# pyannote/pyannote-audio

Measured on AMD Instinct MI355X. Metric: audio-hours/sec (real-time factor) for speaker-diarization-3.1 pipeline, higher is better.
Workload: dtype f32

## Files before the change

include/pyannote_amd.h:

```cpp
#ifndef PYANNOTE_AMD_H
#define PYANNOTE_AMD_H

#include <stddef.h>
#include <stdint.h>

#ifdef __cplusplus
extern "C" {
#endif

int pa_version(void);
const char* pa_last_error(void);

void pa_prof_enable(int on);
size_t pa_prof_report(char* buf, size_t cap);

#define PA_MAX_LSTM_LAYERS 8
#define PA_MAX_LINEAR 4

typedef struct pa_seg_weights {
  int32_t sinc_stride;
  int32_t lstm_layers;
  int32_t lstm_hidden;
  int32_t lstm_bidir;
  int32_t num_linear;
// ... 71 lines not shown
  int32_t bottleneck;
  const float* fb_window;
  const float* fb_tw256;
  const float* fb_tw512;
  const float* fb_mel_w;
  const int32_t* fb_mel_lo;
  const int32_t* fb_mel_hi;
  const float* stem_w;
  const float* stem_shift;
  const float* blk_w1[PA_MAX_RES_BLOCKS];
  const float* blk_shift1[PA_MAX_RES_BLOCKS];
  const float* blk_w2[PA_MAX_RES_BLOCKS];
  const float* blk_shift2[PA_MAX_RES_BLOCKS];
  const float* blk_u1[PA_MAX_RES_BLOCKS];
  const float* blk_u2[PA_MAX_RES_BLOCKS];
  const float* blk_wsc[PA_MAX_RES_BLOCKS];
  const float* blk_shiftsc[PA_MAX_RES_BLOCKS];
  const float* blk_w3[PA_MAX_RES_BLOCKS];
  const float* blk_shift3[PA_MAX_RES_BLOCKS];
  const float* seg1_w;
  const float* seg1_b;
  const float* blk_v1[PA_MAX_RES_BLOCKS];
  const float* blk_v2[PA_MAX_RES_BLOCKS];
  int32_t fb_center_kernel;
} pa_emb_weights;

int pa_emb_num_fbank_frames(int num_samples);
int pa_emb_num_pool_frames(const pa_emb_weights* w, int num_samples);
size_t pa_emb_workspace_bytes(const pa_emb_weights* w, int num_chunks, int num_samples, int num_masks);
int pa_emb_forward(const pa_emb_weights* w, const float* wav, int64_t wav_len, int64_t chunk_stride,
                   int num_chunks, int num_samples, const float* masks, int num_masks, int mask_frames,
                   const int32_t* nearest_idx, float* emb, void* workspace, size_t workspace_bytes,
                   void* stream);

size_t pa_emb_ragged_workspace_bytes(const pa_emb_weights* w, int num_utterances, int max_samples);
int pa_emb_forward_ragged(const pa_emb_weights* w, const float* wav, int64_t wav_len, const int64_t* offsets,
                          const int32_t* lengths, int num_utterances, int max_samples, const float* masks, float* emb,
                          void* workspace, size_t workspace_bytes, void* stream);

size_t pa_emb_calibrate_workspace_bytes(const pa_emb_weights* w, int num_chunks, int num_samples);
int pa_emb_calibrate_winograd(const pa_emb_weights* w, const float* wav, int64_t wav_len, int64_t chunk_stride,
                              int num_chunks, int num_samples, float* report, float* emb, void* workspace,
                              size_t workspace_bytes, void* stream);
int pa_absmax_diff(const float* got, const float* ref, long n, float* out2, void* stream);

int pa_fbank(const float* wav, long wav_len, long chunk_stride, int B, int N, const float* window,
             const float* tw256, const float* tw512, const float* mel_w, const int* mel_lo,
             const int* mel_hi, int nmel, float* out, int center, void* stream);
int pa_fbank_center_span(const float* fb, int B, int T, int nmel, int kernel, float* out, void* stream);
int pa_resnet_stem(const float* fbank, int B, int T, int F, const float* w9, const float* shift,
                   float* out, void* stream);
int pa_conv3x3(const float* X, int B, int H, int W, int cin, const float* Wg, const float* shift,
               const float* R, float* Y, int cout, int stride, int relu, void* stream);
int pa_winograd_pack_host(const float* conv_weight ,
                          const float* bn_scale , int cout, int cin,
                          float* U_slabs );
int pa_conv3x3_wino(const float* X, int B, int H, int W, int cin, const float* U, const float* shift,
                    const float* R, float* Y, int cout, int relu, void* stream);
int pa_winograd4_pack_host(const float* conv_weight ,
                           const float* bn_scale , int cout, int cin,
                           float* U_slabs );
int pa_conv3x3_wino4(const float* X, int B, int H, int W, int cin, const float* U, const float* shift,
                     const float* R, float* Y, int cout, int relu, void* stream);
int pa_conv3x3_wino4_rows(const float* X, int B, int H, int W, int cin, const float* U, const float* shift,
                          const float* R, float* Y, int cout, int relu, int rows, void* stream);
int pa_conv3x3_wino_rows(const float* X, int B, int H, int W, int cin, const float* U, const float* shift,
                         const float* R, float* Y, int cout, int relu, int y_first, void* stream);
int pa_stats_pool(const float* feat, int B, int Fh, int Tp, int C, const float* masks, int S, int Fm,
                  const int* nearest_idx, float* stats, void* stream);
int pa_fbank_ragged(const float* wav, long wav_len, const int64_t* offsets, const int32_t* lengths, int B,
                    int max_samples, const float* window, const float* tw256, const float* tw512, const float* mel_w,
                    const int* mel_lo, const int* mel_hi, int nmel, float* out, void* stream);
int pa_zero_tail_cols(float* x, int B, int H, int W, int C, const int32_t* lengths, int halvings, void* stream);
int pa_stats_pool_ragged(const float* feat, int B, int Fh, int W, int C, const int32_t* lengths, int halvings,
                         const float* masks, int ld_masks, float* stats, void* stream);

#define PA_W2V_MAX_CONV 8
#define PA_W2V_MAX_LAYERS 24
typedef struct pa_w2v_layer {
  const float* qk_w;
  const float* qk_b;
  const float* v_w;
  const float* out_w;
  const float* out_b;
  const float* ln1_g;
  const float* ln1_b;
  const float* ff1_w;
  const float* ff1_b;
  const float* ff2_w;
  const float* ff2_b;
  const float* ln2_g;
  const float* ln2_b;
  const float* gate_w;
  const float* gate_b;
  const float* gate_const;
} pa_w2v_layer;

typedef struct pa_sser_weights {
  int32_t num_conv;
  int32_t conv_channels[PA_W2V_MAX_CONV];
  int32_t conv_kernel[PA_W2V_MAX_CONV];
  int32_t conv_stride[PA_W2V_MAX_CONV];
  int32_t extractor_layer_norm;
  int32_t embed_dim, num_layers, num_heads, ff_dim, layer_norm_first;
  int32_t pos_kernel, pos_groups;
  int32_t wavlm;
// ... 238 lines not shown
```

pyannote-audio_amd/csrc/emb_forward.cpp:

```cpp
#include "forward_common.h"

namespace {

struct EmbPlan {
  int B, N, T, F, S;
  int Hs[5], Ws[5];
  size_t fbank, act[4], stats, total, act_elems;
  size_t t2_off, gather_off;
};

inline bool prefer_wino4(int H, int W, int cin) {
  auto up = [](int a, int b) { return (long)((a + b - 1) / b) * b; };
  long p4 = up(H, 4) * up(W, 64);
  const long p4_lin = up(H, 4) * up(W, 4);
  if (p4_lin * 120 <= p4 * 100) p4 = p4_lin * 120 / 100;
  long p2 = up(H, 8) * up(W, 32);
  if (up(H, 4) * up(W, 64) < p2) p2 = up(H, 4) * up(W, 64);
  if (up(H, 2) * up(W, 128) < p2) p2 = up(H, 2) * up(W, 128);
  const long gain = cin >= 256 ? 130 : 122;
  return p4 * 100 <= p2 * gain;
}

bool make_plan(const pa_emb_weights* w, int B, int N, int S, EmbPlan* p, bool calib = false) {
  if (N < 400) return false;
  p->B = B;
  p->N = N;
  p->S = S < 1 ? 1 : S;
  p->T = 1 + (N - 400) / 160;
  p->F = w->num_mel;
  p->Hs[0] = p->F;
  p->Ws[0] = p->T;
  for (int l = 0; l < w->num_layers; ++l) {
    const int s = l == 0 ? 1 : 2;
    p->Hs[l + 1] = (p->Hs[l] - 1) / s + 1;
    p->Ws[l + 1] = (p->Ws[l] - 1) / s + 1;
  }
  pa::Bump ws;
  p->fbank = ws.take((size_t)B * p->T * p->F);
  const int ex = w->bottleneck ? 4 : 1;
  p->act_elems = (size_t)B * p->Hs[0] * p->Ws[0] * w->planes[0] * ex;
  for (int i = 0; i < 3; ++i) p->act[i] = ws.take(p->act_elems);
  p->t2_off = p->gather_off = 0;
  if (w->bottleneck) {
    size_t t1 = 0, t2 = 0, g = 0;
    int cin = w->planes[0];
    for (int l = 0; l < w->num_layers; ++l) {
      const size_t planes = w->planes[l];
      const size_t in_px = (size_t)B * p->Hs[l == 0 ? 1 : l] * p->Ws[l == 0 ? 1 : l];
      const size_t out_px = (size_t)B * p->Hs[l + 1] * p->Ws[l + 1];
      t1 = t1 > in_px * planes ? t1 : in_px * planes;
      t2 = t2 > out_px * planes ? t2 : out_px * planes;
      if (l > 0) g = g > out_px * cin ? g : out_px * cin;
      cin = 4 * (int)planes;
// ... 50 lines not shown
    pa::set_error("pa_emb_forward: workspace too small (%zu < %zu bytes)", workspace_bytes,
                  p.total * sizeof(float));
    return 3;
  }
  float* ws = (float*)workspace;
  const int B = p.B;

  const int span = w->fb_center_kernel;
  if (ragged && span != 0) {
    pa::set_error("pa_emb_forward_ragged: fbank_centering_span checkpoints run one launch sequence per length");
    return 3;
  }
  if (ragged)
    PA_RUN(pa_fbank_ragged(wav, wav_len, offsets, lengths, B, p.N, w->fb_window, w->fb_tw256, w->fb_tw512, w->fb_mel_w,
                           w->fb_mel_lo, w->fb_mel_hi, w->num_mel, ws + p.fbank, stream));
  else
    PA_RUN(pa_fbank(wav, wav_len, chunk_stride, B, p.N, w->fb_window, w->fb_tw256, w->fb_tw512, w->fb_mel_w,
                    w->fb_mel_lo, w->fb_mel_hi, w->num_mel, ws + p.fbank, span == 0 ? 1 : 0, stream));
  auto zero_tail = [&](float* X, int l, int C) -> int {
    return ragged ? pa_zero_tail_cols(X, B, p.Hs[l], p.Ws[l], C, lengths, l > 0 ? l - 1 : 0, stream) : 0;
  };
  float* cur = ws + p.act[0];
  float* f1 = ws + p.act[1];
  float* f2 = ws + p.act[2];
  const float* feats = ws + p.fbank;
  if (span != 0) {
    PA_RUN(pa_fbank_center_span(ws + p.fbank, B, p.T, p.F, span, f1, stream));
    feats = f1;
  }
  PA_RUN(pa_resnet_stem(feats, B, p.T, p.F, w->stem_w, w->stem_shift, cur, stream));
  if (!w->bottleneck) PA_RUN(zero_tail(cur, 0, w->planes[0]));

  auto conv_s1 = [&](const float* X, int H, int W, int ci, const float* v, const float* u, const float* wd,
                     const float* shift, const float* R, float* Y, int co, int slot) -> int {
    if (calib != nullptr) {
      float* scratch = ws + p.act[3];
      float* rep = calib + 4 * slot;
      const long n = (long)B * H * W * co;
      int r = pa_conv3x3(X, B, H, W, ci, wd, shift, R, Y, co, 1, 1, stream);
      if (r == 0 && v != nullptr) {
        r = pa_conv3x3_wino4(X, B, H, W, ci, v, shift, R, scratch, co, 1, stream);
        if (r == 0) r = pa_absmax_diff(scratch, Y, n, rep, stream);
      }
      if (r == 0 && u != nullptr) {
        r = pa_conv3x3_wino(X, B, H, W, ci, u, shift, R, scratch, co, 1, stream);
        if (r == 0) r = pa_absmax_diff(scratch, Y, n, rep + 2, stream);
      }
      return r;
    }
    if (v != nullptr && prefer_wino4(H, W, ci)) return pa_conv3x3_wino4(X, B, H, W, ci, v, shift, R, Y, co, 1, stream);
    if (u != nullptr) return pa_conv3x3_wino(X, B, H, W, ci, u, shift, R, Y, co, 1, stream);
    return pa_conv3x3(X, B, H, W, ci, wd, shift, R, Y, co, 1, 1, stream);
  };

  int blk = 0;
  int cin = w->planes[0];
  if (w->bottleneck) {
    float* nxt = f1;
    float* sc = f2;
    float* tmp = ws + p.act[3];
    for (int l = 0; l < w->num_layers; ++l) {
      const int planes = w->planes[l], cout = 4 * planes;
      for (int i = 0; i < w->num_blocks[l]; ++i, ++blk) {
        if (blk >= PA_MAX_RES_BLOCKS) {
          pa::set_error("pa_emb_forward: more than %d residual blocks", PA_MAX_RES_BLOCKS);
          return 3;
        }
        const int stride = (i == 0 && l > 0) ? 2 : 1;
        const int H = stride == 2 ? p.Hs[l] : p.Hs[l + 1], W = stride == 2 ? p.Ws[l] : p.Ws[l + 1];
        const int Ho = p.Hs[l + 1], Wo = p.Ws[l + 1];
        float* t1 = tmp;
        float* t2 = tmp + p.t2_off;
        PA_RUN(pa_gemm_tn_ex(cur, cin, w->blk_w1[blk], cin, w->blk_shift1[blk], nullptr, t1, planes, B * H * W,
                             planes, cin, 2, 0, stream));
        PA_RUN(zero_tail(t1, stride == 2 ? l : l + 1, planes));
        if (stride == 1 && w->blk_u2[blk] != nullptr)
          PA_RUN(pa_conv3x3_wino(t1, B, H, W, planes, w->blk_u2[blk], w->blk_shift2[blk], nullptr, t2, planes, 1,
                                 stream));
        else
          PA_RUN(pa_conv3x3(t1, B, H, W, planes, w->blk_w2[blk], w->blk_shift2[blk], nullptr, t2, planes, stride,
                            1, stream));
        const float* res = cur;
        if (w->blk_wsc[blk] != nullptr) {
          if (stride == 2)
            PA_RUN(pa_gemm_tn_s2(cur, B, H, W, cin, w->blk_wsc[blk], cin, w->blk_shiftsc[blk], sc, cout, cout, stream));
          else
            PA_RUN(pa_gemm_tn_ex(cur, cin, w->blk_wsc[blk], cin, w->blk_shiftsc[blk], nullptr, sc, cout,
                                 B * Ho * Wo, cout, cin, 0, 0, stream));
          res = sc;
        } else if (stride != 1 || cin != cout) {
          pa::set_error("pa_emb_forward: block %d needs a shortcut conv but none was given", blk);
          return 3;
        }
        PA_RUN(pa_gemm_tn_ex(t2, planes, w->blk_w3[blk], planes, w->blk_shift3[blk], res, nxt, cout, B * Ho * Wo,
                             cout, planes, 2, 0, stream));
        float* t = cur;
        cur = nxt;
        nxt = t;
        cin = cout;
      }
    }
  } else
  for (int l = 0; l < w->num_layers; ++l) {
    const int cout = w->planes[l];
    for (int i = 0; i < w->num_blocks[l]; ++i, ++blk) {
      if (blk >= PA_MAX_RES_BLOCKS) {
        pa::set_error("pa_emb_forward: more than %d residual blocks", PA_MAX_RES_BLOCKS);
        return 3;
      }
      const int stride = (i == 0 && l > 0) ? 2 : 1;
      const int H = stride == 2 ? p.Hs[l] : p.Hs[l + 1], W = stride == 2 ? p.Ws[l] : p.Ws[l + 1];
      const int Ho = p.Hs[l + 1], Wo = p.Ws[l + 1];
      if (w->blk_wsc[blk] != nullptr) {
        PA_RUN(pa_conv3x3(cur, B, H, W, cin, w->blk_w1[blk], w->blk_shift1[blk], nullptr, f1, cout, stride,
                          1, stream));
        PA_RUN(zero_tail(f1, l + 1, cout));
        const size_t q = (size_t)B * Ho * Wo * cin;
        float* R = f2 + pa::Bump::align(q);
        if (stride == 2)
          PA_RUN(pa_gemm_tn_s2(cur, B, H, W, cin, w->blk_wsc[blk], cin, w->blk_shiftsc[blk], R, cout, cout, stream));
        else
          PA_RUN(pa_gemm_tn(cur, cin, w->blk_wsc[blk], cin, w->blk_shiftsc[blk], R, cout, B * Ho * Wo, cout, cin, 0, 0,
                            stream));
        PA_RUN(conv_s1(f1, Ho, Wo, cout, w->blk_v2[blk], w->blk_u2[blk], w->blk_w2[blk], w->blk_shift2[blk], R, cur,
                       cout, 2 * blk + 1));
        PA_RUN(zero_tail(cur, l + 1, cout));
      } else {
        if (stride != 1 || cin != cout) {
          pa::set_error("pa_emb_forward: block %d needs a shortcut conv but none was given", blk);
          return 3;
        }
        PA_RUN(conv_s1(cur, H, W, cin, w->blk_v1[blk], w->blk_u1[blk], w->blk_w1[blk], w->blk_shift1[blk], nullptr, f1,
                       cout, 2 * blk));
        PA_RUN(zero_tail(f1, l + 1, cout));
        PA_RUN(conv_s1(f1, H, W, cout, w->blk_v2[blk], w->blk_u2[blk], w->blk_w2[blk], w->blk_shift2[blk], cur, f2,
                       cout, 2 * blk + 1));
        PA_RUN(zero_tail(f2, l + 1, cout));
        float* t = cur;
        cur = f2;
        f2 = t;
      }
      cin = cout;
    }
  }
  const int L = w->num_layers;
  const int S = p.S;
  const int cfin = w->planes[L - 1] * (w->bottleneck ? 4 : 1);
  if (ragged)
    PA_RUN(pa_stats_pool_ragged(cur, B, p.Hs[L], p.Ws[L], cfin, lengths, L - 1, masks, p.Ws[L], ws + p.stats, stream));
  else
    PA_RUN(pa_stats_pool(cur, B, p.Hs[L], p.Ws[L], cfin, masks, S, mask_frames, nearest_idx, ws + p.stats, stream));
  const int D2 = 2 * cfin * p.Hs[L];
  PA_RUN(pa_gemm_tn(ws + p.stats, D2, w->seg1_w, D2, w->seg1_b, emb, w->embed_dim, B * S, w->embed_dim, D2,
                    0, 0, stream));
  return 0;
}

extern "C" {

int pa_emb_forward(const pa_emb_weights* w, const float* wav, int64_t wav_len, int64_t chunk_stride,
                   int num_chunks, int num_samples, const float* masks, int num_masks, int mask_frames,
                   const int32_t* nearest_idx, float* emb, void* workspace, size_t workspace_bytes,
                   void* stream) {
  return emb_forward_impl(w, wav, wav_len, chunk_stride, num_chunks, num_samples, masks, num_masks, mask_frames,
                          nearest_idx, emb, workspace, workspace_bytes, stream, nullptr);
}

size_t pa_emb_ragged_workspace_bytes(const pa_emb_weights* w, int num_utterances, int max_samples) {
  EmbPlan p;
  if (!make_plan(w, num_utterances, max_samples, 1, &p)) return 0;
  return p.total * sizeof(float);
}

int pa_emb_forward_ragged(const pa_emb_weights* w, const float* wav, int64_t wav_len, const int64_t* offsets,
// ... 30 lines not shown
```

pyannote-audio_amd/csrc/emb_resnet.hip:

```cpp
#include "common.h"

namespace pa {

constexpr int STEM_TS = 64;
constexpr int STEM_LD = STEM_TS + 3;

__global__ __launch_bounds__(256) void k_stem(const float* __restrict__ fb, int T, int F,
                                              const float* __restrict__ w9,
                                              const float* __restrict__ shift,
                                              float* __restrict__ out) {
  extern __shared__ float xs[];
  const int b = blockIdx.y, t0 = blockIdx.x * STEM_TS;
  const int tid = threadIdx.x;
  for (int i = tid; i < 2 * STEM_LD; i += 256) xs[(i < STEM_LD ? 0 : (F + 1) * STEM_LD - STEM_LD) + i] = 0.f;
  const int n = (STEM_TS + 2) * F;
  for (int i0 = 0; i0 < n; i0 += 8 * 256) {
    float v[8];
#pragma unroll
    for (int k = 0; k < 8; ++k) {
      const int i = i0 + tid + 256 * k;
      const int tt = i / F, ff = i - tt * F, t = t0 + tt - 1;
      v[k] = (i < n && t >= 0 && t < T) ? fb[((long)b * T + t) * F + ff] : 0.f;
    }
#pragma unroll
// ... 24 lines not shown
  float* o = out + ((long)b * F * T + t0 + pl) * 32 + q4;
  for (int f = 0; f < F; ++f) {
#pragma unroll
    for (int h = 0; h < 2; ++h)
#pragma unroll
      for (int dt = 0; dt < 3; ++dt) x2[h][dt] = xs[(f + 2) * STEM_LD + pl + 32 * h + dt];
    float* of = o + (long)f * T * 32;
#pragma unroll
    for (int h = 0; h < 2; ++h) {
      float acc[4];
#pragma unroll
      for (int c = 0; c < 4; ++c) acc[c] = 0.f;
#pragma unroll
      for (int dt = 0; dt < 3; ++dt)
#pragma unroll
        for (int c = 0; c < 4; ++c) acc[c] = fmaf(x0[h][dt], w[dt][c], acc[c]);
#pragma unroll
      for (int dt = 0; dt < 3; ++dt)
#pragma unroll
        for (int c = 0; c < 4; ++c) acc[c] = fmaf(x1[h][dt], w[3 + dt][c], acc[c]);
#pragma unroll
      for (int dt = 0; dt < 3; ++dt)
#pragma unroll
        for (int c = 0; c < 4; ++c) acc[c] = fmaf(x2[h][dt], w[6 + dt][c], acc[c]);
      float4 o4;
      o4.x = fmaxf(acc[0] + sh[0], 0.f);
      o4.y = fmaxf(acc[1] + sh[1], 0.f);
      o4.z = fmaxf(acc[2] + sh[2], 0.f);
      o4.w = fmaxf(acc[3] + sh[3], 0.f);
      if (h == 0 ? ok0 : ok1) *reinterpret_cast<float4*>(of + 32 * 32 * h) = o4;
    }
#pragma unroll
    for (int h = 0; h < 2; ++h)
#pragma unroll
      for (int dt = 0; dt < 3; ++dt) {
        x0[h][dt] = x1[h][dt];
        x1[h][dt] = x2[h][dt];
      }
  }
}

constexpr int CB = 16;
constexpr int CLD = CB + 4;

template <int S, int TH, int TWT>
struct ConvGeom {
  static constexpr int TW = 32 * TWT;
  static constexpr int PH = (TH - 1) * S + 3;
  static constexpr int PW = (TW - 1) * S + 3;
  static constexpr int PWH = ((TW + 1 + 3) / 8) * 8 + 4;
  static constexpr int PATCH = S == 1 ? PH * PW * CLD : PH * 2 * PWH * CLD;
};

template <int S, int TH, int TWT, int BN, bool HAS_R>
__global__ __launch_bounds__(256, 2) void k_conv3x3(const float* __restrict__ X, int H, int W, int CIN,
                                                    const float* __restrict__ Wg,
                                                    const float* __restrict__ shift,
                                                    const float* __restrict__ R, float* __restrict__ Y,
                                                    int Ho, int Wo, int COUT, int relu, int tiles_w,
                                                    int tiles_hw, int n_tiles, int total_tiles, int xranges,
                                                    int* __restrict__ counters) {
  using G = ConvGeom<S, TH, TWT>;
  constexpr int MT = TH * TWT;
  constexpr int MPW = MT / 4;
  constexpr int NT = BN / 32;
  static_assert(MT % 4 == 0, "M-tiles must split over 4 waves");
  extern __shared__ __attribute__((aligned(16))) float smem[];
  float* patch = smem;
  float* wts = smem + G::PATCH;

  const int tid = threadIdx.x, lane = tid & 63, wv = tid >> 6;
  const int li = lane & 31, kh = lane >> 5;
  constexpr int NPF4 = G::PH * G::PW * (CB / 4);
  constexpr int NP = (NPF4 + 255) / 256;
  constexpr int NWF4 = 9 * BN * (CB / 4);
  constexpr int NW = (NWF4 + 255) / 256;
  constexpr int OOB = (int)0x80000000;

  struct Tile {
    int b, n0, y0, x0;
  };
  const int num_pb = total_tiles / n_tiles;
  auto pair_of = [&](int t) {
    return xranges ? (t & 7) * ((num_pb + 7) >> 3) + (t >> 3) / n_tiles : ((t >> 3) / n_tiles) * 8 + (t & 7);
  };
  auto decode = [&](int t) {
    Tile q;
    const int pb = pair_of(t);
    q.n0 = (((t >> 3) % n_tiles)) * BN;
    const int pix = pb % tiles_hw;
    q.b = pb / tiles_hw;
    q.y0 = (pix / tiles_w) * TH;
    q.x0 = (pix % tiles_w) * G::TW;
    return q;
  };
  auto resolve = [&](const TileQueue& tqq, int r) {
    for (;;) {
      const int t = tq_resolve(tqq, r);
      if (t < 0 || pair_of(t) < num_pb) return t;
      r = tq_claim_own(tqq);
    }
  };
  u32x4 rp[NP], rw[NW];
  constexpr bool HOIST = S == 2;
  struct Offs {
    int p[NP];
  };
  int offw[NW];
#pragma unroll
  for (int e = 0; e < NW; ++e) {
    const int i = tid + 256 * e;
    const int c4 = i & 3, rn = i >> 2;
    const int tap = rn / BN, n = rn % BN;
    offw[e] = (NWF4 % 256 == 0 || i < NWF4) ? ((tap * COUT + n) * CIN + 4 * c4) * 4 : OOB;
  }
  auto tile_offsets = [&](const Tile& q, Offs& o) {
#pragma unroll
    for (int e = 0; e < NP; ++e) {
      const int i = tid + 256 * e;
      const int c4 = i & 3, pp = i >> 2;
      const int py = pp / G::PW, px = pp % G::PW;
      const int iy = q.y0 * S - 1 + py, ix = q.x0 * S - 1 + px;
      o.p[e] = ((NPF4 % 256 == 0 || i < NPF4) && iy >= 0 && iy < H && ix >= 0 && ix < W)
                   ? ((iy * W + ix) * CIN + 4 * c4) * 4
                   : OOB;
    }
  };
  auto gload = [&](const Tile& q, const Offs& o, int c0) {
    const __amdgpu_buffer_rsrc_t xsrd = __builtin_amdgcn_make_buffer_rsrc(
        const_cast<float*>(X + (long)q.b * H * W * CIN), 0, H * W * CIN * 4, 0x00020000);
    const __amdgpu_buffer_rsrc_t wsrd = __builtin_amdgcn_make_buffer_rsrc(
        const_cast<float*>(Wg + (long)q.n0 * CIN), 0, (9 * COUT - q.n0) * CIN * 4, 0x00020000);
    Offs here;
    if (!HOIST) tile_offsets(q, here);
#pragma unroll
    for (int e = 0; e < NP; ++e)
      rp[e] = __builtin_amdgcn_raw_buffer_load_b128(xsrd, HOIST ? o.p[e] : here.p[e], c0 * 4, 0);
#pragma unroll
    for (int e = 0; e < NW; ++e) rw[e] = __builtin_amdgcn_raw_buffer_load_b128(wsrd, offw[e], c0 * 4, 0);
  };
  auto lstore = [&]() {
#pragma unroll
    for (int e = 0; e < NP; ++e) {
      const int i = tid + 256 * e;
      const int c4 = i & 3, pp = i >> 2;
      const int py = pp / G::PW, px = pp % G::PW;
      int off;
      if (S == 1) off = pp * CLD + 4 * c4;
      else off = ((py * 2 + (px & 1)) * G::PWH + (px >> 1)) * CLD + 4 * c4;
      if (NPF4 % 256 == 0 || i < NPF4) *reinterpret_cast<u32x4*>(patch + off) = rp[e];
    }
#pragma unroll
    for (int e = 0; e < NW; ++e) {
      const int i = tid + 256 * e;
      if (NWF4 % 256 == 0 || i < NWF4)
        *reinterpret_cast<u32x4*>(wts + (i >> 2) * CLD + 4 * (i & 3)) = rw[e];
    }
  };

  __shared__ int s_next;
  const TileQueue tq{counters, (int)(blockIdx.x & 7), ((num_pb + 7) >> 3) * n_tiles};
  if (tid == 0) s_next = resolve(tq, tq_claim_own(tq));
  __syncthreads();
  int t = s_next;
  if (t < 0) {
    if (tid == 0) tq_done(tq, gridDim.x);
    return;
  }
  Tile cur = decode(t);
  Offs oc, on;
  if (HOIST) tile_offsets(cur, oc);
  on = oc;
  gload(cur, oc, 0);
  for (;;) {
    int ahead = 0;
    if (tid == 0) ahead = tq_claim_own(tq);
    int tn = -1;
    f32x16 acc[MPW][NT];
#pragma unroll
    for (int i = 0; i < MPW; ++i)
#pragma unroll
      for (int j = 0; j < NT; ++j)
#pragma unroll
        for (int r = 0; r < 16; ++r) acc[i][j][r] = 0.f;
    Tile nxt = cur;

    for (int c0 = 0; c0 < CIN; c0 += CB) {
      __syncthreads();
      lstore();
      if (c0 == 0 && tid == 0) s_next = resolve(tq, ahead);
      __syncthreads();
      if (c0 == 0) {
        tn = s_next;
        if (tn >= 0) {
          nxt = decode(tn);
          if (HOIST) tile_offsets(nxt, on);
        }
      }
      if (c0 + CB < CIN) gload(cur, oc, c0 + CB);
      else if (tn >= 0) gload(nxt, on, 0);
      float4 af[1][MPW][2], bf[1][NT][2];
      auto load_tap = [&](int tap, float4 (&a)[MPW][2], float4 (&bq)[NT][2]) {
        const int dy = tap / 3, dx = tap % 3;
#pragma unroll
        for (int i = 0; i < MPW; ++i) {
          const int mt = wv * MPW + i;
          const int yy = mt / TWT, xt = mt % TWT;
          int off;
          if (S == 1) off = ((yy + dy) * G::PW + 32 * xt + li + dx) * CLD;
          else off = (((yy * 2 + dy) * 2 + (dx & 1)) * G::PWH + 32 * xt + li + (dx >> 1)) * CLD;
          a[i][0] = *reinterpret_cast<const float4*>(patch + off + kh * 8);
          a[i][1] = *reinterpret_cast<const float4*>(patch + off + kh * 8 + 4);
        }
#pragma unroll
        for (int j = 0; j < NT; ++j) {
          const int off = (tap * BN + 32 * j + li) * CLD + kh * 8;
          bq[j][0] = *reinterpret_cast<const float4*>(wts + off);
          bq[j][1] = *reinterpret_cast<const float4*>(wts + off + 4);
        }
      };
      auto mfma_tap = [&](const float4 (&a)[MPW][2], const float4 (&bq)[NT][2]) {
#pragma unroll
        for (int h = 0; h < 2; ++h)
#pragma unroll
          for (int i = 0; i < MPW; ++i)
#pragma unroll
            for (int j = 0; j < NT; ++j) {
              acc[i][j] = MFMA32(a[i][h].x, bq[j][h].x, acc[i][j]);
              acc[i][j] = MFMA32(a[i][h].y, bq[j][h].y, acc[i][j]);
              acc[i][j] = MFMA32(a[i][h].z, bq[j][h].z, acc[i][j]);
              acc[i][j] = MFMA32(a[i][h].w, bq[j][h].w, acc[i][j]);
            }
      };
#pragma unroll 1
      for (int dy = 0; dy < 3; ++dy)
#pragma unroll
        for (int dx = 0; dx < 3; ++dx) {
          load_tap(dy * 3 + dx, af[0], bf[0]);
          mfma_tap(af[0], bf[0]);
        }
    }
    {
      const __amdgpu_buffer_rsrc_t ysrd = __builtin_amdgcn_make_buffer_rsrc(
          Y + (long)cur.b * Ho * Wo * COUT, 0, Ho * Wo * COUT * 4, 0x00020000);
      const __amdgpu_buffer_rsrc_t rsrd = __builtin_amdgcn_make_buffer_rsrc(
          const_cast<float*>(HAS_R ? R + (long)cur.b * Ho * Wo * COUT : Y), 0,
          Ho * Wo * COUT * 4, 0x00020000);
      constexpr int NG = MPW * NT;
      int off[2][16];
      float rv[2][16];
      auto goffs = [&](int g, int* o) {
        const int i = g / NT, j = g % NT;
        const int mt = wv * MPW + i;
        const int y = cur.y0 + mt / TWT, xbase = cur.x0 + 32 * (mt % TWT) + 4 * kh;
        const int n = cur.n0 + 32 * j + li;
#pragma unroll
        for (int r = 0; r < 16; ++r) {
          const int x = xbase + (r & 3) + 8 * (r >> 2);
          o[r] = (y < Ho && x < Wo) ? ((y * Wo + x) * COUT + n) * 4 : OOB;
        }
      };
      auto gres = [&](const int* o, float* v) {
        if (HAS_R) {
#pragma unroll
          for (int r = 0; r < 16; ++r)
            v[r] = __builtin_bit_cast(float, __builtin_amdgcn_raw_buffer_load_b32(rsrd, o[r], 0, 0));
        } else {
#pragma unroll
          for (int r = 0; r < 16; ++r) v[r] = 0.f;
        }
      };
      goffs(0, off[0]);
      gres(off[0], rv[0]);
#pragma unroll
      for (int g = 0; g < NG; ++g) {
        if (g + 1 < NG) {
          goffs(g + 1, off[(g + 1) & 1]);
          gres(off[(g + 1) & 1], rv[(g + 1) & 1]);
        }
        const int i = g / NT, j = g % NT;
        const float sh = shift[cur.n0 + 32 * j + li];
#pragma unroll
        for (int r = 0; r < 16; ++r) {
          float v = acc[i][j][r] + sh + rv[g & 1][r];
          if (relu) v = fmaxf(v, 0.f);
          __builtin_amdgcn_raw_buffer_store_b32(__builtin_bit_cast(unsigned int, v), ysrd, off[g & 1][r], 0, 0);
        }
      }
    }
    if (tn < 0) break;
    cur = nxt;
    oc = on;
  }
  if (tid == 0) tq_done(tq, gridDim.x);
}

int xcd_ranges_wanted(bool by_default);

template <int S, int TH, int TWT, int BN, bool HAS_R>
static int launch_conv_r(const float* X, int B, int H, int W, int CIN, const float* Wg,
                         const float* shift, const float* R, float* Y, int COUT, int relu,
                         hipStream_t st) {
  using G = ConvGeom<S, TH, TWT>;
  const int Ho = (H - 1) / S + 1, Wo = (W - 1) / S + 1;
  const int tiles_w = cdiv(Wo, G::TW), tiles_h = cdiv(Ho, TH);
  const size_t lds = (size_t)(G::PATCH + 9 * BN * CLD) * sizeof(float);
  constexpr int MAXDEV = 16;
  static int resident_of[MAXDEV] = {0}, per_cu_of[MAXDEV] = {0};
  int dev = 0;
  (void)hipGetDevice(&dev);
  if (dev < 0 || dev >= MAXDEV) dev = 0;
  if (!resident_of[dev]) {
    (void)hipFuncSetAttribute((const void*)k_conv3x3<S, TH, TWT, BN, HAS_R>,
                              hipFuncAttributeMaxDynamicSharedMemorySize, (int)lds);
    int cus = 256, per_cu = 2;
    (void)hipDeviceGetAttribute(&cus, hipDeviceAttributeMultiprocessorCount, dev);
    if (hipOccupancyMaxActiveBlocksPerMultiprocessor(&per_cu, k_conv3x3<S, TH, TWT, BN, HAS_R>, 256, lds) !=
            hipSuccess || per_cu < 1)
      per_cu = 2;
    resident_of[dev] = cus * per_cu;
    per_cu_of[dev] = per_cu;
  }
  const int resident = resident_of[dev] & ~7;
  const int tiles_hw = tiles_w * tiles_h, n_tiles = COUT / BN;
  const long total = (long)tiles_hw * n_tiles * B;
  const int grid = (int)(total < resident ? total : resident);
  int* counters = tile_counters();
  if (counters == nullptr) {
    set_error("pa_conv3x3: cannot allocate the tile counters");
    return 2;
  }
  hipLaunchKernelGGL((k_conv3x3<S, TH, TWT, BN, HAS_R>), dim3(grid), dim3(256), lds, st, X, H, W, CIN, Wg,
                     shift, R, Y, Ho, Wo, COUT, relu, tiles_w, tiles_hw, n_tiles, (int)total, xcd_ranges_wanted(true),
                     counters);
  return 0;
}

template <int S, int TH, int TWT, int BN>
static int launch_conv(const float* X, int B, int H, int W, int CIN, const float* Wg,
                       const float* shift, const float* R, float* Y, int COUT, int relu,
                       hipStream_t st) {
  return R != nullptr ? launch_conv_r<S, TH, TWT, BN, true>(X, B, H, W, CIN, Wg, shift, R, Y, COUT, relu, st)
                      : launch_conv_r<S, TH, TWT, BN, false>(X, B, H, W, CIN, Wg, shift, R, Y, COUT, relu, st);
}

}

extern "C" {

int pa_resnet_stem(const float* fbank, int B, int T, int F, const float* w9, const float* shift,
                   float* out, void* stream) {
  if (B <= 0) return 0;
  pa::ProfScope prof("k_stem", stream, 2.0 * B * T * F * 9 * 32, 4.0 * B * T * F * 33);
  PA_REQUIRE(F >= 1 && (size_t)(F + 2) * pa::STEM_LD * 4 <= 64 * 1024, "pa_resnet_stem: %d mel bins do not fit LDS", F);
  hipLaunchKernelGGL(pa::k_stem, dim3(pa::cdiv(T, pa::STEM_TS), B), dim3(256), (size_t)(F + 2) * pa::STEM_LD * 4,
                     (hipStream_t)stream, fbank, T, F, w9, shift, out);
  PA_CHECK_LAUNCH("pa_resnet_stem");
  return 0;
}

int pa_conv3x3(const float* X, int B, int H, int W, int cin, const float* Wg, const float* shift,
               const float* R, float* Y, int cout, int stride, int relu, void* stream) {
  if (B <= 0) return 0;
  PA_REQUIRE(cin % pa::CB == 0 && cout % 32 == 0, "pa_conv3x3: cin %% 16 and cout %% 32 required");
  hipStream_t st = (hipStream_t)stream;
  const int Ho = (H - 1) / stride + 1, Wo_ = (W - 1) / stride + 1;
  pa::ProfScope prof("k_conv3x3", stream, 2.0 * 9 * cin * cout * (double)B * Ho * Wo_,
                     4.0 * ((double)B * H * W * cin + (double)B * Ho * Wo_ * cout * (R ? 2 : 1) + 9.0 * cin * cout));
  if (stride == 1) {
    if (cout == 32) pa::launch_conv<1, 8, 1, 32>(X, B, H, W, cin, Wg, shift, R, Y, cout, relu, st);
    else if (Ho >= 32) pa::launch_conv<1, 8, 1, 64>(X, B, H, W, cin, Wg, shift, R, Y, cout, relu, st);
    else if (Ho >= 16) pa::launch_conv<1, 4, 2, 64>(X, B, H, W, cin, Wg, shift, R, Y, cout, relu, st);
    else pa::launch_conv<1, 2, 2, 64>(X, B, H, W, cin, Wg, shift, R, Y, cout, relu, st);
  } else if (stride == 2) {
    PA_REQUIRE(cout % 64 == 0, "pa_conv3x3: stride 2 needs cout %% 64 == 0");
    if (Ho >= 16) pa::launch_conv<2, 4, 1, 32>(X, B, H, W, cin, Wg, shift, R, Y, cout, relu, st);
    else pa::launch_conv<2, 2, 2, 32>(X, B, H, W, cin, Wg, shift, R, Y, cout, relu, st);
  } else {
    PA_REQUIRE(false, "pa_conv3x3: stride %d not supported", stride);
  }
  PA_CHECK_LAUNCH("pa_conv3x3");
  return 0;
}

}
```

pyannote-audio_amd/ffi.py:

```python
from __future__ import annotations

import ctypes as C
from pathlib import Path

import torch

_LIB = None
PA_MAX_LSTM_LAYERS = 8
PA_MAX_LINEAR = 4

c_fp = C.c_void_p


class SegWeights(C.Structure):
    _fields_ = [
        ("sinc_stride", C.c_int32), ("lstm_layers", C.c_int32), ("lstm_hidden", C.c_int32),
        ("lstm_bidir", C.c_int32), ("num_linear", C.c_int32), ("linear_hidden", C.c_int32),
        ("num_classes", C.c_int32), ("num_speakers", C.c_int32),
        ("wav_gamma", C.c_float), ("wav_beta", C.c_float),
        ("sinc_filt", c_fp), ("norm0", c_fp), ("conv1_w", c_fp), ("conv1_b", c_fp), ("norm1", c_fp),
        ("conv2_w", c_fp), ("conv2_b", c_fp), ("norm2", c_fp),
        ("lstm_wih", c_fp * PA_MAX_LSTM_LAYERS), ("lstm_bias", c_fp * PA_MAX_LSTM_LAYERS),
        ("lstm_whh", c_fp * PA_MAX_LSTM_LAYERS),
        ("lin_w", c_fp * PA_MAX_LINEAR), ("lin_b", c_fp * PA_MAX_LINEAR),
# ... 125 lines not shown
    lib.pa_sinc_fix_pool.argtypes = [c_fp, C.c_long, C.c_int, C.c_int, C.c_int, c_fp, c_fp, C.c_float, C.c_float,
                                     c_fp, c_fp, c_fp, c_fp]
    lib.pa_sinc_fir_span_centred.argtypes = [c_fp, C.c_long, C.c_long, c_fp, c_fp, c_fp, c_fp, c_fp]
    lib.pa_sinc_fix_pool_centred.argtypes = [c_fp, C.c_long, C.c_int, C.c_int, C.c_int, c_fp, C.c_long, C.c_int, c_fp,
                                             c_fp, C.c_float, C.c_float, c_fp, c_fp, c_fp, c_fp]
    lib.pa_conv5_pool.argtypes = [c_fp, C.c_int, C.c_int, C.c_int, c_fp, c_fp, c_fp, c_fp, c_fp, c_fp,
                                  c_fp, c_fp]
    lib.pa_norm_transpose.argtypes = [c_fp, C.c_int, C.c_int, c_fp, c_fp, c_fp, c_fp, c_fp, c_fp]
    lib.pa_gemm_tn_ex.argtypes = [c_fp, C.c_int, c_fp, C.c_int, c_fp, c_fp, c_fp, C.c_long, C.c_int, C.c_int,
                                  C.c_int, C.c_int, C.c_int, c_fp]
    lib.pa_gemm_tn.argtypes = [c_fp, C.c_int, c_fp, C.c_int, c_fp, c_fp, C.c_long, C.c_int, C.c_int,
                               C.c_int, C.c_int, C.c_int, c_fp]
    lib.pa_lstm_rec.argtypes = [c_fp, c_fp, c_fp, C.c_int, C.c_int, C.c_int, c_fp]
    lib.pa_classifier.argtypes = [c_fp, C.c_int, C.c_int, C.c_int, C.c_int, C.c_int, c_fp, c_fp,
                                  C.c_int, c_fp, C.c_int, c_fp, c_fp, c_fp]
    lib.pa_prof_enable.argtypes = [C.c_int]
    lib.pa_prof_enable.restype = None
    lib.pa_prof_report.argtypes = [C.c_char_p, C.c_size_t]
    lib.pa_prof_report.restype = C.c_size_t
    _declare_optional(lib)
    _LIB = lib
    return lib


_OPTIONAL: list[tuple] = [
    ("pa_emb_num_fbank_frames", [C.c_int], C.c_int),
    ("pa_emb_num_pool_frames", [C.POINTER(EmbWeights), C.c_int], C.c_int),
    ("pa_emb_workspace_bytes", [C.POINTER(EmbWeights), C.c_int, C.c_int, C.c_int], C.c_size_t),
    ("pa_emb_forward", [C.POINTER(EmbWeights), c_fp, C.c_int64, C.c_int64, C.c_int, C.c_int, c_fp,
                        C.c_int, C.c_int, c_fp, c_fp, c_fp, C.c_size_t, c_fp], C.c_int),
    ("pa_emb_ragged_workspace_bytes", [C.POINTER(EmbWeights), C.c_int, C.c_int], C.c_size_t),
    ("pa_emb_forward_ragged", [C.POINTER(EmbWeights), c_fp, C.c_int64, c_fp, c_fp, C.c_int, C.c_int, c_fp, c_fp,
                               c_fp, C.c_size_t, c_fp], C.c_int),
    ("pa_fbank_ragged", [c_fp, C.c_long, c_fp, c_fp, C.c_int, C.c_int, c_fp, c_fp, c_fp, c_fp, c_fp, c_fp, C.c_int,
                         c_fp, c_fp], C.c_int),
    ("pa_zero_tail_cols", [c_fp, C.c_int, C.c_int, C.c_int, C.c_int, c_fp, C.c_int, c_fp], C.c_int),
    ("pa_stats_pool_ragged", [c_fp, C.c_int, C.c_int, C.c_int, C.c_int, c_fp, C.c_int, c_fp, C.c_int, c_fp, c_fp],
     C.c_int),
    ("pa_emb_calibrate_workspace_bytes", [C.POINTER(EmbWeights), C.c_int, C.c_int], C.c_size_t),
    ("pa_emb_calibrate_winograd", [C.POINTER(EmbWeights), c_fp, C.c_int64, C.c_int64, C.c_int, C.c_int, c_fp, c_fp,
                                   c_fp, C.c_size_t, c_fp], C.c_int),
    ("pa_lstm_rec_h", [c_fp, c_fp, c_fp, C.c_int, C.c_int, C.c_int, C.c_int, c_fp], C.c_int),
    ("pa_absmax_diff", [c_fp, c_fp, C.c_long, c_fp, c_fp], C.c_int),
    ("pa_gemm_tn_s2", [c_fp, C.c_int, C.c_int, C.c_int, C.c_int, c_fp, C.c_int, c_fp, c_fp, C.c_long, C.c_int,
                       c_fp], C.c_int),
    ("pa_gemm_tn_batched", [c_fp, C.c_int, C.c_long, C.c_long, c_fp, C.c_int, C.c_long, C.c_long, c_fp, c_fp, C.c_long,
                            C.c_long, C.c_long, C.c_int, C.c_int, C.c_int, C.c_int, C.c_int, C.c_int, c_fp], C.c_int),
    ("pa_fbank", [c_fp, C.c_long, C.c_long, C.c_int, C.c_int, c_fp, c_fp, c_fp, c_fp, c_fp, c_fp,
                  C.c_int, c_fp, C.c_int, c_fp], C.c_int),
    ("pa_fbank_center_span", [c_fp, C.c_int, C.c_int, C.c_int, C.c_int, c_fp, c_fp], C.c_int),
    ("pa_resnet_stem", [c_fp, C.c_int, C.c_int, C.c_int, c_fp, c_fp, c_fp, c_fp], C.c_int),
    ("pa_conv3x3", [c_fp, C.c_int, C.c_int, C.c_int, C.c_int, c_fp, c_fp, c_fp, c_fp, C.c_int, C.c_int,
                    C.c_int, c_fp], C.c_int),
    ("pa_conv3x3_wino", [c_fp, C.c_int, C.c_int, C.c_int, C.c_int, c_fp, c_fp, c_fp, c_fp, C.c_int, C.c_int,
                         c_fp], C.c_int),
    ("pa_conv3x3_wino4", [c_fp, C.c_int, C.c_int, C.c_int, C.c_int, c_fp, c_fp, c_fp, c_fp, C.c_int, C.c_int,
                          c_fp], C.c_int),
    ("pa_conv3x3_wino4_rows", [c_fp, C.c_int, C.c_int, C.c_int, C.c_int, c_fp, c_fp, c_fp, c_fp, C.c_int, C.c_int,
                               C.c_int, c_fp], C.c_int),
    ("pa_conv3x3_wino_rows", [c_fp, C.c_int, C.c_int, C.c_int, C.c_int, c_fp, c_fp, c_fp, c_fp, C.c_int, C.c_int,
                              C.c_int, c_fp], C.c_int),
    ("pa_pdist_f64", [c_fp, C.c_int, C.c_int, c_fp, c_fp], C.c_int),
    ("pa_cdist_cosine_f64", [c_fp, C.c_int, c_fp, C.c_int, C.c_int, c_fp, c_fp, c_fp], C.c_int),
    ("pa_centroid_means", [c_fp, C.c_int, c_fp, c_fp, C.c_int, c_fp, c_fp], C.c_int),
    ("pa_linkage_workspace_bytes", [C.c_int], C.c_size_t),
    ("pa_linkage_centroid_f64", [c_fp, C.c_int, c_fp, c_fp, C.c_size_t, c_fp], C.c_int),
    ("pa_linkage_centroid_f64_ex", [c_fp, C.c_int, c_fp, c_fp, C.c_size_t, C.c_int, c_fp], C.c_int),
    ("pa_pdist_cosine_f64", [c_fp, C.c_int, C.c_int, c_fp, c_fp, c_fp], C.c_int),
    ("pa_nonfinite_flag_f64", [c_fp, C.c_long, c_fp, c_fp], C.c_int),
    ("pa_linkage_chain_workspace_bytes", [C.c_int], C.c_size_t),
    ("pa_linkage_chain_f64", [c_fp, C.c_int, C.c_int, c_fp, c_fp, C.c_size_t, c_fp], C.c_int),
    ("pa_seg_chunk_stats", [c_fp, C.c_int, C.c_int, C.c_int, c_fp, c_fp, c_fp], C.c_int),
    ("pa_embedding_masks", [c_fp, C.c_int, C.c_int, C.c_int, c_fp, C.c_int, C.c_int, c_fp, c_fp], C.c_int),
    ("pa_speaker_count", [c_fp, C.c_int, C.c_int, C.c_int, c_fp, C.c_int, c_fp, c_fp, c_fp], C.c_int),
    ("pa_cluster_activations", [c_fp, C.c_int, C.c_int, C.c_int, c_fp, c_fp, C.c_int, C.c_int, c_fp, c_fp],
     C.c_int),
    ("pa_topk_binarize", [c_fp, c_fp, C.c_int, C.c_int, C.c_int, c_fp, c_fp, c_fp], C.c_int),
    ("pa_topk_binarize_f32", [c_fp, c_fp, C.c_int, C.c_int, C.c_int, c_fp, c_fp, c_fp], C.c_int),
    ("pa_binarize_hysteresis", [c_fp, C.c_int, C.c_int, C.c_int, C.c_float, C.c_float, C.c_int, c_fp, c_fp],
     C.c_int),
    ("pa_cluster_max", [c_fp, C.c_int, C.c_int, C.c_int, c_fp, C.c_int, c_fp, c_fp], C.c_int),
    ("pa_aggregate", [c_fp, C.c_int, C.c_int, C.c_int, c_fp, C.c_int, c_fp, c_fp, C.c_float, C.c_float, C.c_int,
                      c_fp, c_fp], C.c_int),
    ("pa_binarize_regions_workspace_bytes", [C.c_int, C.c_int, C.c_int], C.c_size_t),
    ("pa_binarize_regions", [c_fp, C.c_int, C.c_int, c_fp, c_fp, c_fp, c_fp, C.c_double, C.c_double, C.c_double,
                             C.c_int, c_fp, c_fp, c_fp, c_fp, C.c_size_t, c_fp], C.c_int),
    ("pa_resample_poly", [c_fp, C.c_long, c_fp, C.c_int, C.c_int, C.c_int, C.c_int, c_fp, C.c_long, c_fp],
     C.c_int),
    ("pa_plda_transform", [c_fp, C.c_int, C.c_int, C.c_int, C.c_int, c_fp, c_fp, c_fp, c_fp, c_fp, c_fp, c_fp],
     C.c_int),
    ("pa_vbx_workspace_bytes", [C.c_int, C.c_int, C.c_int], C.c_size_t),
    ("pa_vbx_iteration", [c_fp, c_fp, C.c_int, C.c_int, C.c_int, C.c_double, C.c_double, C.c_int, c_fp, c_fp,
                          c_fp, C.c_size_t, c_fp], C.c_int),
    ("pa_stats_pool", [c_fp, C.c_int, C.c_int, C.c_int, C.c_int, c_fp, C.c_int, C.c_int, c_fp, c_fp,
                       c_fp], C.c_int),
    ("pa_stats_pool_rows", [c_fp, C.c_int, C.c_int, C.c_int, C.c_int, C.c_int, c_fp, C.c_int, C.c_int, c_fp,
                            c_fp, C.c_int, c_fp, c_fp, c_fp], C.c_int),
    ("pa_sser_num_frames", [C.POINTER(SserWeights), C.c_int], C.c_int),
    ("pa_sser_workspace_bytes", [C.POINTER(SserWeights), C.c_int, C.c_int], C.c_size_t),
    ("pa_sser_forward", [C.POINTER(SserWeights), c_fp, C.c_int64, C.c_int64, C.c_int, C.c_int, c_fp, c_fp, c_fp,
                         c_fp, C.c_size_t, c_fp], C.c_int),
    ("pa_w2v_conv0", [c_fp, C.c_long, C.c_long, C.c_int, C.c_int, C.c_int, C.c_int, C.c_int, C.c_int, C.c_int, c_fp,
                      c_fp, c_fp, c_fp], C.c_int),
    ("pa_w2v_group_norm_gelu", [c_fp, C.c_int, C.c_int, C.c_int, C.c_int, c_fp, c_fp, c_fp, c_fp, c_fp], C.c_int),
    ("pa_w2v_layernorm", [c_fp, c_fp, C.c_long, C.c_int, c_fp, c_fp, C.c_int, c_fp], C.c_int),
    ("pa_w2v_posconv", [c_fp, C.c_int, C.c_int, C.c_int, C.c_int, C.c_int, C.c_int, c_fp, c_fp, c_fp, c_fp], C.c_int),
# ... 106 lines not shown
```

Measured before the change: 1.308.

## Fuse stride-2 1x1 shortcut GEMM into the block-entry 3x3 conv kernel

At stride-2 residual block entries, the 1x1 projection shortcut is now computed inside the 3x3 conv kernel as a tenth weight tap reusing the centre-tap activations already in LDS, writing both outputs. This removes a separate shortcut GEMM launch and its second read of the input activations. In exchange it adds a second accumulator set (more registers) and extra LDS for the shortcut weights, which may reduce occupancy. It can be disabled with the PA_ENTRY_FUSED environment variable.

New measurement: 1.319, median of 6. No clear change (+0.8%).

```diff
diff --git a/include/pyannote_amd.h b/include/pyannote_amd.h
--- a/include/pyannote_amd.h
+++ b/include/pyannote_amd.h
@@ -147,6 +147,8 @@
                    float* out, void* stream);
 int pa_conv3x3(const float* X, int B, int H, int W, int cin, const float* Wg, const float* shift,
                const float* R, float* Y, int cout, int stride, int relu, void* stream);
+int pa_conv3x3_s2_sc(const float* X, int B, int H, int W, int cin, const float* Wg, const float* shift,
+                     const float* Wsc, const float* shift_sc, float* Y, float* Ysc, int cout, int relu, void* stream);
 int pa_winograd_pack_host(const float* conv_weight ,
                           const float* bn_scale , int cout, int cin,
                           float* U_slabs );
diff --git a/pyannote-audio_amd/csrc/emb_forward.cpp b/pyannote-audio_amd/csrc/emb_forward.cpp
--- a/pyannote-audio_amd/csrc/emb_forward.cpp
+++ b/pyannote-audio_amd/csrc/emb_forward.cpp
@@ -1,4 +1,6 @@
 #include "forward_common.h"
+
+#include <cstdlib>
 
 namespace {
 
@@ -155,6 +157,9 @@
     if (u != nullptr) return pa_conv3x3_wino(X, B, H, W, ci, u, shift, R, Y, co, 1, stream);
     return pa_conv3x3(X, B, H, W, ci, wd, shift, R, Y, co, 1, 1, stream);
   };
+
+  const char* entry_env = getenv("PA_ENTRY_FUSED");
+  const bool entry_fused = entry_env == nullptr || atoi(entry_env) != 0;
 
   int blk = 0;
   int cin = w->planes[0];
@@ -215,14 +220,19 @@
       const int H = stride == 2 ? p.Hs[l] : p.Hs[l + 1], W = stride == 2 ? p.Ws[l] : p.Ws[l + 1];
       const int Ho = p.Hs[l + 1], Wo = p.Ws[l + 1];
       if (w->blk_wsc[blk] != nullptr) {
-        PA_RUN(pa_conv3x3(cur, B, H, W, cin, w->blk_w1[blk], w->blk_shift1[blk], nullptr, f1, cout, stride,
-                          1, stream));
-        PA_RUN(zero_tail(f1, l + 1, cout));
         const size_t q = (size_t)B * Ho * Wo * cin;
         float* R = f2 + pa::Bump::align(q);
-        if (stride == 2)
+        const bool fused = stride == 2 && entry_fused;
+        if (fused)
+          PA_RUN(pa_conv3x3_s2_sc(cur, B, H, W, cin, w->blk_w1[blk], w->blk_shift1[blk], w->blk_wsc[blk],
+                                  w->blk_shiftsc[blk], f1, R, cout, 1, stream));
+        else
+          PA_RUN(pa_conv3x3(cur, B, H, W, cin, w->blk_w1[blk], w->blk_shift1[blk], nullptr, f1, cout, stride,
+                            1, stream));
+        PA_RUN(zero_tail(f1, l + 1, cout));
+        if (stride == 2 && !fused)
           PA_RUN(pa_gemm_tn_s2(cur, B, H, W, cin, w->blk_wsc[blk], cin, w->blk_shiftsc[blk], R, cout, cout, stream));
-        else
+        else if (stride != 2)
           PA_RUN(pa_gemm_tn(cur, cin, w->blk_wsc[blk], cin, w->blk_shiftsc[blk], R, cout, B * Ho * Wo, cout, cin, 0, 0,
                             stream));
         PA_RUN(conv_s1(f1, Ho, Wo, cout, w->blk_v2[blk], w->blk_u2[blk], w->blk_w2[blk], w->blk_shift2[blk], R, cur,
diff --git a/pyannote-audio_amd/csrc/emb_resnet.hip b/pyannote-audio_amd/csrc/emb_resnet.hip
--- a/pyannote-audio_amd/csrc/emb_resnet.hip
+++ b/pyannote-audio_amd/csrc/emb_resnet.hip
@@ -100,19 +100,24 @@
   static constexpr int PATCH = S == 1 ? PH * PW * CLD : PH * 2 * PWH * CLD;
 };
 
-template <int S, int TH, int TWT, int BN, bool HAS_R>
+template <int S, int TH, int TWT, int BN, bool HAS_R, bool SC = false>
 __global__ __launch_bounds__(256, 2) void k_conv3x3(const float* __restrict__ X, int H, int W, int CIN,
                                                     const float* __restrict__ Wg,
                                                     const float* __restrict__ shift,
                                                     const float* __restrict__ R, float* __restrict__ Y,
                                                     int Ho, int Wo, int COUT, int relu, int tiles_w,
                                                     int tiles_hw, int n_tiles, int total_tiles, int xranges,
-                                                    int* __restrict__ counters) {
+                                                    int* __restrict__ counters,
+                                                    const float* __restrict__ Wsc,
+                                                    const float* __restrict__ shift_sc,
+                                                    float* __restrict__ Ysc) {
   using G = ConvGeom<S, TH, TWT>;
   constexpr int MT = TH * TWT;
   constexpr int MPW = MT / 4;
   constexpr int NT = BN / 32;
   static_assert(MT % 4 == 0, "M-tiles must split over 4 waves");
+  static_assert(!SC || (S == 2 && !HAS_R && BN % 16 == 0), "the shortcut rides along the stride-2 block entry only");
+  constexpr int NTAP = SC ? 10 : 9;
   extern __shared__ __attribute__((aligned(16))) float smem[];
   float* patch = smem;
   float* wts = smem + G::PATCH;
@@ -121,7 +126,7 @@
   const int li = lane & 31, kh = lane >> 5;
   constexpr int NPF4 = G::PH * G::PW * (CB / 4);
   constexpr int NP = (NPF4 + 255) / 256;
-  constexpr int NWF4 = 9 * BN * (CB / 4);
+  constexpr int NWF4 = NTAP * BN * (CB / 4);
   constexpr int NW = (NWF4 + 255) / 256;
   constexpr int OOB = (int)0x80000000;
 
@@ -161,7 +166,9 @@
     const int c4 = i & 3, rn = i >> 2;
     const int tap = rn / BN, n = rn % BN;
     offw[e] = (NWF4 % 256 == 0 || i < NWF4) ? ((tap * COUT + n) * CIN + 4 * c4) * 4 : OOB;
-  }
+    if (SC && tap == 9) offw[e] = (n * CIN + 4 * c4) * 4;
+  }
+  const int wvu = SC ? __builtin_amdgcn_readfirstlane(wv) : 0;
   auto tile_offsets = [&](const Tile& q, Offs& o) {
 #pragma unroll
     for (int e = 0; e < NP; ++e) {
@@ -185,7 +192,19 @@
     for (int e = 0; e < NP; ++e)
       rp[e] = __builtin_amdgcn_raw_buffer_load_b128(xsrd, HOIST ? o.p[e] : here.p[e], c0 * 4, 0);
 #pragma unroll
-    for (int e = 0; e < NW; ++e) rw[e] = __builtin_amdgcn_raw_buffer_load_b128(wsrd, offw[e], c0 * 4, 0);
+    for (int e = 0; e < NW; ++e) {
+      if constexpr (SC) {
+        if (((256 * e + 255) >> 2) / BN >= 9) {
+          const bool sc_rows = ((256 * e + 64 * wvu) >> 2) / BN >= 9;
+          const __amdgpu_buffer_rsrc_t srd = __builtin_amdgcn_make_buffer_rsrc(
+              const_cast<float*>((sc_rows ? Wsc : Wg) + (long)q.n0 * CIN), 0,
+              ((sc_rows ? COUT : 9 * COUT) - q.n0) * CIN * 4, 0x00020000);
+          rw[e] = __builtin_amdgcn_raw_buffer_load_b128(srd, offw[e], c0 * 4, 0);
+          continue;
+        }
+      }
+      rw[e] = __builtin_amdgcn_raw_buffer_load_b128(wsrd, offw[e], c0 * 4, 0);
+    }
   };
   auto lstore = [&]() {
 #pragma unroll
@@ -231,6 +250,15 @@
       for (int j = 0; j < NT; ++j)
 #pragma unroll
         for (int r = 0; r < 16; ++r) acc[i][j][r] = 0.f;
+    f32x16 accs[SC ? MPW : 1][SC ? NT : 1];
+    if constexpr (SC) {
+#pragma unroll
+      for (int i = 0; i < MPW; ++i)
+#pragma unroll
+        for (int j = 0; j < NT; ++j)
+#pragma unroll
+          for (int r = 0; r < 16; ++r) accs[i][j][r] = 0.f;
+    }
     Tile nxt = cur;
 
     for (int c0 = 0; c0 < CIN; c0 += CB) {
@@ -286,6 +314,27 @@
         for (int dx = 0; dx < 3; ++dx) {
           load_tap(dy * 3 + dx, af[0], bf[0]);
           mfma_tap(af[0], bf[0]);
+          if constexpr (SC) {
+            if (dy == 1 && dx == 1) {
+#pragma unroll
+              for (int j = 0; j < NT; ++j) {
+                const int off = (9 * BN + 32 * j + li) * CLD + kh * 8;
+                bf[0][j][0] = *reinterpret_cast<const float4*>(wts + off);
+                bf[0][j][1] = *reinterpret_cast<const float4*>(wts + off + 4);
+              }
+#pragma unroll
+              for (int h = 0; h < 2; ++h)
+#pragma unroll
+                for (int i = 0; i < MPW; ++i)
+#pragma unroll
+                  for (int j = 0; j < NT; ++j) {
+                    accs[i][j] = MFMA32(af[0][i][h].x, bf[0][j][h].x, accs[i][j]);
+                    accs[i][j] = MFMA32(af[0][i][h].y, bf[0][j][h].y, accs[i][j]);
+                    accs[i][j] = MFMA32(af[0][i][h].z, bf[0][j][h].z, accs[i][j]);
+                    accs[i][j] = MFMA32(af[0][i][h].w, bf[0][j][h].w, accs[i][j]);
+                  }
+            }
+          }
         }
     }
     {
@@ -335,6 +384,20 @@
           __builtin_amdgcn_raw_buffer_store_b32(__builtin_bit_cast(unsigned int, v), ysrd, off[g & 1][r], 0, 0);
         }
       }
+      if constexpr (SC) {
+        const __amdgpu_buffer_rsrc_t ssrd = __builtin_amdgcn_make_buffer_rsrc(
+            Ysc + (long)cur.b * Ho * Wo * COUT, 0, Ho * Wo * COUT * 4, 0x00020000);
+#pragma unroll
+        for (int g = 0; g < NG; ++g) {
+          goffs(g, off[0]);
+          const int i = g / NT, j = g % NT;
+          const float sh = shift_sc[cur.n0 + 32 * j + li];
+#pragma unroll
+          for (int r = 0; r < 16; ++r)
+            __builtin_amdgcn_raw_buffer_store_b32(__builtin_bit_cast(unsigned int, accs[i][j][r] + sh), ssrd, off[0][r],
+                                                  0, 0);
+        }
+      }
     }
     if (tn < 0) break;
     cur = nxt;
@@ -345,29 +408,34 @@
 
 int xcd_ranges_wanted(bool by_default);
 
-template <int S, int TH, int TWT, int BN, bool HAS_R>
+template <int S, int TH, int TWT, int BN, bool HAS_R, bool SC = false>
 static int launch_conv_r(const float* X, int B, int H, int W, int CIN, const float* Wg,
                          const float* shift, const float* R, float* Y, int COUT, int relu,
-                         hipStream_t st) {
+                         hipStream_t st, const float* Wsc = nullptr, const float* shift_sc = nullptr,
+                         float* Ysc = nullptr) {
   using G = ConvGeom<S, TH, TWT>;
   const int Ho = (H - 1) / S + 1, Wo = (W - 1) / S + 1;
   const int tiles_w = cdiv(Wo, G::TW), tiles_h = cdiv(Ho, TH);
-  const size_t lds = (size_t)(G::PATCH + 9 * BN * CLD) * sizeof(float);
+  const size_t lds = (size_t)(G::PATCH + (SC ? 10 : 9) * BN * CLD) * sizeof(float);
   constexpr int MAXDEV = 16;
   static int resident_of[MAXDEV] = {0}, per_cu_of[MAXDEV] = {0};
   int dev = 0;
   (void)hipGetDevice(&dev);
   if (dev < 0 || dev >= MAXDEV) dev = 0;
   if (!resident_of[dev]) {
-    (void)hipFuncSetAttribute((const void*)k_conv3x3<S, TH, TWT, BN, HAS_R>,
+    (void)hipFuncSetAttribute((const void*)k_conv3x3<S, TH, TWT, BN, HAS_R, SC>,
                               hipFuncAttributeMaxDynamicSharedMemorySize, (int)lds);
     int cus = 256, per_cu = 2;
     (void)hipDeviceGetAttribute(&cus, hipDeviceAttributeMultiprocessorCount, dev);
-    if (hipOccupancyMaxActiveBlocksPerMultiprocessor(&per_cu, k_conv3x3<S, TH, TWT, BN, HAS_R>, 256, lds) !=
+    if (hipOccupancyMaxActiveBlocksPerMultiprocessor(&per_cu, k_conv3x3<S, TH, TWT, BN, HAS_R, SC>, 256, lds) !=
             hipSuccess || per_cu < 1)
       per_cu = 2;
     resident_of[dev] = cus * per_cu;
     per_cu_of[dev] = per_cu;
+  }
+  if (SC && per_cu_of[dev] < 2) {
+    set_error("pa_conv3x3_s2_sc: %d workgroup per CU with %zu B of LDS, 2 required", per_cu_of[dev], lds);
+    return 2;
   }
   const int resident = resident_of[dev] & ~7;
   const int tiles_hw = tiles_w * tiles_h, n_tiles = COUT / BN;
@@ -378,9 +446,9 @@
     set_error("pa_conv3x3: cannot allocate the tile counters");
     return 2;
   }
-  hipLaunchKernelGGL((k_conv3x3<S, TH, TWT, BN, HAS_R>), dim3(grid), dim3(256), lds, st, X, H, W, CIN, Wg,
+  hipLaunchKernelGGL((k_conv3x3<S, TH, TWT, BN, HAS_R, SC>), dim3(grid), dim3(256), lds, st, X, H, W, CIN, Wg,
                      shift, R, Y, Ho, Wo, COUT, relu, tiles_w, tiles_hw, n_tiles, (int)total, xcd_ranges_wanted(true),
-                     counters);
+                     counters, Wsc, shift_sc, Ysc);
   return 0;
 }
 
@@ -431,4 +499,24 @@
   return 0;
 }
 
-}
+int pa_conv3x3_s2_sc(const float* X, int B, int H, int W, int cin, const float* Wg, const float* shift,
+                     const float* Wsc, const float* shift_sc, float* Y, float* Ysc, int cout, int relu, void* stream) {
+  if (B <= 0) return 0;
+  PA_REQUIRE(cin % pa::CB == 0 && cout % 64 == 0, "pa_conv3x3_s2_sc: cin %% 16 and cout %% 64 required");
+  hipStream_t st = (hipStream_t)stream;
+  const int Ho = (H - 1) / 2 + 1, Wo_ = (W - 1) / 2 + 1;
+  pa::ProfScope prof("k_conv3x3", stream, 2.0 * 10 * cin * cout * (double)B * Ho * Wo_,
+                     4.0 * ((double)B * H * W * cin + 2.0 * B * Ho * Wo_ * cout + 10.0 * cin * cout));
+  int rc;
+  if (Ho >= 16)
+    rc = pa::launch_conv_r<2, 4, 1, 32, false, true>(X, B, H, W, cin, Wg, shift, nullptr, Y, cout, relu, st, Wsc,
+                                                      shift_sc, Ysc);
+  else
+    rc = pa::launch_conv_r<2, 2, 2, 32, false, true>(X, B, H, W, cin, Wg, shift, nullptr, Y, cout, relu, st, Wsc,
+                                                      shift_sc, Ysc);
+  if (rc != 0) return rc;
+  PA_CHECK_LAUNCH("pa_conv3x3_s2_sc");
+  return 0;
+}
+
+}
diff --git a/pyannote-audio_amd/ffi.py b/pyannote-audio_amd/ffi.py
--- a/pyannote-audio_amd/ffi.py
+++ b/pyannote-audio_amd/ffi.py
@@ -201,6 +201,8 @@
     ("pa_resnet_stem", [c_fp, C.c_int, C.c_int, C.c_int, c_fp, c_fp, c_fp, c_fp], C.c_int),
     ("pa_conv3x3", [c_fp, C.c_int, C.c_int, C.c_int, C.c_int, c_fp, c_fp, c_fp, c_fp, C.c_int, C.c_int,
                     C.c_int, c_fp], C.c_int),
+    ("pa_conv3x3_s2_sc", [c_fp, C.c_int, C.c_int, C.c_int, C.c_int, c_fp, c_fp, c_fp, c_fp, c_fp, c_fp, C.c_int,
+                          C.c_int, c_fp], C.c_int),
     ("pa_conv3x3_wino", [c_fp, C.c_int, C.c_int, C.c_int, C.c_int, c_fp, c_fp, c_fp, c_fp, C.c_int, C.c_int,
                          c_fp], C.c_int),
     ("pa_conv3x3_wino4", [c_fp, C.c_int, C.c_int, C.c_int, C.c_int, c_fp, c_fp, c_fp, c_fp, C.c_int, C.c_int,
```
